# barbararoessle/e2e_multi_view_matching

Hardware: NVIDIA H100
Metric: view-tuples/sec @1024 kpts 5-view (higher is better)
Workload: dtype f32 via split operands on the tensor cores (fp16x3 / tf32x3, fp32-faithful) / f64 pose kernels

## Files before the change

### e2e_multi_view_matching_b200/csrc/attention_h3.cu

```cuda
#include "attention_wg.cuh"

int g_attn_h3_variant = 1;
extern "C" void mvm_debug_set_attention_h3_variant(int v) { g_attn_h3_variant = v ? 1 : 0; }

int launch_attention_h3(const float* qkv, const __half* kh, const __half* kl, const __half* vh, const __half* vl,
                        float* out, int batch, int n_pad, AttnSegs segs, int is_cross, cudaStream_t stream) {
  MVM_REQUIRE(qkv && kh && kl && vh && vl && out);
  MVM_REQUIRE(n_pad % 64 == 0 && attn_segs_valid(segs, n_pad, is_cross));
  MvmProfScope prof__(MVM_TAG_ATTN, stream);
  const long long rows = (long long)batch * segs.n_views * n_pad;
  const CUtensorMap* tK = mvm_get_tmap_2d_f16(kh, rows, 256, 256, attn_wg::BKV);
  const CUtensorMap* tKlo = mvm_get_tmap_2d_f16(kl, rows, 256, 256, attn_wg::BKV);
  const CUtensorMap* tV = mvm_get_tmap_2d_f16(vh, rows, 256, 256, attn_wg::BKV);
  const CUtensorMap* tVlo = mvm_get_tmap_2d_f16(vl, rows, 256, 256, attn_wg::BKV);
  return attn_wg::launch<16>(tK, tV, tKlo, tVlo, qkv, out, batch, n_pad, segs, is_cross, stream);
}
```

### e2e_multi_view_matching_b200/csrc/attention_tc.cu

```cuda
#include "attention_wg.cuh"

long long* g_attn_dbg = nullptr;

extern "C" void mvm_debug_set_attention_timing(long long* buf) { g_attn_dbg = buf; }

int launch_attention_tc(const float* qkv, const float* vt, float* out, int batch, int n_pad, AttnSegs segs,
                        int is_cross, int n_pass, cudaStream_t stream, const float* klo, const float* vtlo) {
  MVM_REQUIRE(n_pad % 64 == 0 && attn_segs_valid(segs, n_pad, is_cross));
  MvmProfScope prof__(MVM_TAG_ATTN, stream);
  const int V = batch * segs.n_views;
  const long long rows = (long long)V * n_pad;
  const CUtensorMap* tK = mvm_get_tmap_2d(qkv, rows, 768, 768, attn_wg::BKV);
  const CUtensorMap* tV = mvm_get_tmap_2d(vt, (long long)V * 256, n_pad, n_pad, attn_wg::HD);
  if (n_pass == 3) {
    MVM_REQUIRE(klo && vtlo);
    const CUtensorMap* tKlo = mvm_get_tmap_2d(klo, rows, 256, 256, attn_wg::BKV);
    const CUtensorMap* tVlo = mvm_get_tmap_2d(vtlo, (long long)V * 256, n_pad, n_pad, attn_wg::HD);
    return attn_wg::launch<3>(tK, tV, tKlo, tVlo, qkv, out, batch, n_pad, segs, is_cross, stream);
  }
  return attn_wg::launch<1>(tK, tV, tK, tV, qkv, out, batch, n_pad, segs, is_cross, stream);
}
```

### e2e_multi_view_matching_b200/csrc/attention_wg.cuh

```cuda
#pragma once
#include <cuda_fp16.h>
#include "common.cuh"
#include "kernels.cuh"
#include "tc_common.cuh"

namespace attn_wg {

constexpr int BQ = 128, BKV = 64, HD = 64;
constexpr int NTHREADS = 288;
constexpr int PRODUCER_WARP = 8;
constexpr int PP_BAR = 1, Q_BAR = 3;

template <int MODE>
struct Cfg {
  static constexpr bool F16 = MODE == 16;
  static constexpr bool PIPE = F16;
  static constexpr int PL = MODE == 1 ? 1 : 2;
  static constexpr int PLANE = F16 ? 8192 : 16384;
  static constexpr int TILE = PL * PLANE;
  static constexpr int ST = MODE == 3 ? 3 : 4;
  static constexpr int OFF_V = ST * TILE;
  static constexpr int OFF_Q = 2 * ST * TILE;
  static constexpr int QPLANE = BQ * 128;
  static constexpr int OFF_BAR = OFF_Q + (F16 ? 2 * QPLANE : 0);
  static constexpr int SMEM_BYTES = OFF_BAR + 256 + 1024;
};

struct Args {
  const float* qkv;
  float* out;
  int n_pad;
  AttnSegs segs;
  int is_cross;
};

__device__ __forceinline__ float ex2_ftz(float x) {
  float y;
  asm("ex2.approx.ftz.f32 %0, %1;" : "=f"(y) : "f"(x));
  return y;
}
__device__ __forceinline__ float tf32_hi(float x) {
  return __uint_as_float((__float_as_uint(x) + 0x1000u) & 0xffffe000u);
}
__device__ __forceinline__ void split_pack(float x0, float x1, uint32_t& hi, uint32_t& lo) {
  const __half2 h = __floats2half2_rn(x0, x1);
  const float2 hf = __half22float2(h);
  const __half2 l = __floats2half2_rn(x0 - hf.x, x1 - hf.y);
  hi = *reinterpret_cast<const uint32_t*>(&h);
  lo = *reinterpret_cast<const uint32_t*>(&l);
}
__device__ __forceinline__ void named_bar_sync(int id, int n) {
  asm volatile("bar.sync %0, %1;" ::"r"(id), "r"(n) : "memory");
}
__device__ __forceinline__ void named_bar_arrive(int id, int n) {
  asm volatile("bar.arrive %0, %1;" ::"r"(id), "r"(n) : "memory");
}
template <int N>
__device__ __forceinline__ void fence_regs(uint32_t (*a)[4]) {
#pragma unroll
  for (int i = 0; i < N; ++i)
#pragma unroll
    for (int e = 0; e < 4; ++e) asm volatile("" : "+r"(a[i][e])::"memory");
}

template <int MODE>
__global__ void __launch_bounds__(NTHREADS, 1)
attention_wg_kernel(const __grid_constant__ CUtensorMap tmK, const __grid_constant__ CUtensorMap tmV,
                    const __grid_constant__ CUtensorMap tmKlo, const __grid_constant__ CUtensorMap tmVlo,
                    const __grid_constant__ Args g) {
  using C_ = Cfg<MODE>;
  constexpr bool F16 = C_::F16, PIPE = C_::PIPE;
  constexpr int ST = C_::ST, PLANE = C_::PLANE, TILE = C_::TILE;
  constexpr int KS = F16 ? 4 : 8;
  extern __shared__ uint8_t smem_raw[];
  uint8_t* smem = reinterpret_cast<uint8_t*>((reinterpret_cast<uintptr_t>(smem_raw) + 1023) & ~uintptr_t(1023));
  uint64_t* bars = reinterpret_cast<uint64_t*>(smem + C_::OFF_BAR);
  uint64_t* k_full = bars;
  uint64_t* k_empty = bars + ST;
  uint64_t* v_full = bars + 2 * ST;
  uint64_t* v_empty = bars + 3 * ST;

  const int warp = threadIdx.x >> 5, lane = threadIdx.x & 31;
  const int q0 = blockIdx.x * BQ;
  const int h = blockIdx.y;
  const int v = blockIdx.z;
  const int T = g.segs.n_views;
  const int t = v % T, b = v / T;
  if (q0 >= g.segs.counts[t]) return;

  if (threadIdx.x == 0) {
    for (int i = 0; i < ST; ++i) {
      tc::mbar_init(k_full + i, 1); tc::mbar_init(k_empty + i, 256);
      tc::mbar_init(v_full + i, 1); tc::mbar_init(v_empty + i, 256);
    }
    tc::fence_barrier_init();
  }
  __syncthreads();

  if (warp == PRODUCER_WARP) {
    if (lane == 0) {
      tc::prefetch_tmap(&tmK); tc::prefetch_tmap(&tmV);
      if (MODE != 1) { tc::prefetch_tmap(&tmKlo); tc::prefetch_tmap(&tmVlo); }
      int j = 0;
      for (int sg = 0; sg < T; ++sg) {
        if (g.is_cross ? (sg == t) : (sg != t)) continue;
        const int cnt = g.segs.counts[sg];
        for (int k0 = 0; k0 < cnt; k0 += BKV, ++j) {
          const int s = j % ST;
          const uint32_t ph = ((j / ST) & 1) ^ 1;
          const int krow = (b * T + sg) * g.n_pad + k0;
          uint8_t* sk = smem + s * TILE;
          uint8_t* sv = smem + C_::OFF_V + s * TILE;
          tc::mbar_wait(k_empty + s, ph);
          tc::mbar_arrive_expect_tx(k_full + s, TILE);
          if (F16) {
            tc::tma_load_2d(sk, &tmK, k_full + s, h * HD, krow);
            tc::tma_load_2d(sk + PLANE, &tmKlo, k_full + s, h * HD, krow);
          } else {
            tc::tma_load_2d(sk, &tmK, k_full + s, 256 + h * HD, krow);
            tc::tma_load_2d(sk + 8192, &tmK, k_full + s, 256 + h * HD + 32, krow);
            if (MODE == 3) {
              tc::tma_load_2d(sk + PLANE, &tmKlo, k_full + s, h * HD, krow);
              tc::tma_load_2d(sk + PLANE + 8192, &tmKlo, k_full + s, h * HD + 32, krow);
            }
          }
          tc::mbar_wait(v_empty + s, ph);
          tc::mbar_arrive_expect_tx(v_full + s, TILE);
          if (F16) {
            tc::tma_load_2d(sv, &tmV, v_full + s, h * HD, krow);
            tc::tma_load_2d(sv + PLANE, &tmVlo, v_full + s, h * HD, krow);
          } else {
            const int vrow = (b * T + sg) * 256 + h * HD;
            tc::tma_load_2d(sv, &tmV, v_full + s, k0, vrow);
            tc::tma_load_2d(sv + 8192, &tmV, v_full + s, k0 + 32, vrow);
            if (MODE == 3) {
              tc::tma_load_2d(sv + PLANE, &tmVlo, v_full + s, k0, vrow);
              tc::tma_load_2d(sv + PLANE + 8192, &tmVlo, v_full + s, k0 + 32, vrow);
            }
          }
        }
      }
    }
    return;
  }

  const int wg = warp >> 2, wq = warp & 3;
  const int gr = lane >> 2, tq = lane & 3;
  const int lrow = wg * 64 + wq * 16 + gr;
  float2 qraw[KS][4];
  {
    const long long total = (long long)gridDim.z * g.n_pad;
    const long long r0 = (long long)v * g.n_pad + q0 + lrow;
    const float* q_r0 = g.qkv + r0 * 768 + h * HD;
    const float* q_r1 = q_r0 + 8 * 768;
    const bool in0 = r0 < total, in1 = r0 + 8 < total;
    const float2 z = make_float2(0.f, 0.f);
#pragma unroll
    for (int kk = 0; kk < KS; ++kk) {
      if (F16) {
        const int c = 16 * kk + 2 * tq;
        qraw[kk][0] = in0 ? __ldg(reinterpret_cast<const float2*>(q_r0 + c)) : z;
        qraw[kk][1] = in1 ? __ldg(reinterpret_cast<const float2*>(q_r1 + c)) : z;
        qraw[kk][2] = in0 ? __ldg(reinterpret_cast<const float2*>(q_r0 + c + 8)) : z;
        qraw[kk][3] = in1 ? __ldg(reinterpret_cast<const float2*>(q_r1 + c + 8)) : z;
      } else {
        const int c = 8 * kk + tq;
        qraw[kk][0] = make_float2(in0 ? __ldg(q_r0 + c) : 0.f, 0.f);
        qraw[kk][1] = make_float2(in1 ? __ldg(q_r1 + c) : 0.f, 0.f);
        qraw[kk][2] = make_float2(in0 ? __ldg(q_r0 + c + 4) : 0.f, 0.f);
        qraw[kk][3] = make_float2(in1 ? __ldg(q_r1 + c + 4) : 0.f, 0.f);
      }
    }
  }
  if constexpr (F16) {
    uint8_t* sq = smem + C_::OFF_Q + lrow * 128 + 4 * tq;
#pragma unroll
    for (int kk = 0; kk < KS; ++kk) {
#pragma unroll
      for (int e = 0; e < 4; ++e) {
        uint32_t hi, lo;
        split_pack(qraw[kk][e].x, qraw[kk][e].y, hi, lo);
        const int off = (e & 1) * 1024 + (((2 * kk + (e >> 1)) ^ gr) << 4);
        *reinterpret_cast<uint32_t*>(sq + off) = hi;
        *reinterpret_cast<uint32_t*>(sq + C_::QPLANE + off) = lo;
      }
    }
    tc::fence_proxy_async();
    named_bar_sync(Q_BAR + wg, 128);
  }

  float o[32];
#pragma unroll
  for (int i = 0; i < 32; ++i) o[i] = 0.f;
  float m_run[2] = {-INFINITY, -INFINITY}, l_run[2] = {0.f, 0.f};
  const float scale_l2e = 0.125f * 1.4426950408889634f;
  const int srcA = (lane & ~3) | (tq >> 1), srcB = srcA + 2;
  float sc[32], fo[2];
  uint32_t qhi[KS][4], qlo[KS][4];
  uint32_t phi[KS][4], plo[KS][4];

  auto prep_s = [&] {
    if constexpr (!F16) {
#pragma unroll
      for (int kk = 0; kk < KS; ++kk) {
#pragma unroll
        for (int e = 0; e < 4; ++e) {
          float x = qraw[kk][e].x;
          asm volatile("" : "+f"(x));
          const float hi = MODE == 3 ? tf32_hi(x) : x;
          qhi[kk][e] = __float_as_uint(hi);
          qlo[kk][e] = __float_as_uint(MODE == 3 ? tf32_hi(x - hi) : 0.f);
        }
      }
    }
#pragma unroll
    for (int i = 0; i < 32; ++i) sc[i] = 0.f;
    tc::fence_acc<64>(sc);
  };
  auto issue_s = [&](int st, uint32_t ph) {
    tc::mbar_wait(k_full + st, ph);
    const uint32_t kb = tc::smem_u32(smem + st * TILE);
    tc::wgmma_fence();
#pragma unroll
    for (int kk = 0; kk < KS; ++kk) {
      if (F16) {
        const uint32_t qb = tc::smem_u32(smem + C_::OFF_Q + wg * 64 * 128) + kk * 32;
        const uint64_t dq = tc::make_sw128_desc(qb), dk = tc::make_sw128_desc(kb + kk * 32);
        tc::wgmma_f16_ss<64>(sc, dq, dk);
        tc::wgmma_f16_ss<64>(sc, dq, tc::make_sw128_desc(kb + PLANE + kk * 32));
        tc::wgmma_f16_ss<64>(sc, tc::make_sw128_desc(qb + C_::QPLANE), dk);
      } else {
        const uint32_t off = (kk >> 2) * 8192 + (kk & 3) * 32;
        const uint64_t dk = tc::make_sw128_desc(kb + off);
        tc::wgmma_tf32_rs<64>(sc, qhi[kk], dk);
        if (MODE == 3) {
          tc::wgmma_tf32_rs<64>(sc, qhi[kk], tc::make_sw128_desc(kb + PLANE + off));
          tc::wgmma_tf32_rs<64>(sc, qlo[kk], dk);
        }
      }
    }
    tc::wgmma_commit();
  };
  auto retire_s = [&](int st) {
    tc::fence_acc<64>(sc);
    if constexpr (!F16) { fence_regs<KS>(qhi); fence_regs<KS>(qlo); }
    tc::mbar_arrive(k_empty + st);
  };
  auto issue_pv = [&](int st, uint32_t ph) {
    tc::mbar_wait(v_full + st, ph);
    const uint32_t vb = tc::smem_u32(smem + C_::OFF_V + st * TILE);
    tc::wgmma_fence();
#pragma unroll
    for (int kk = 0; kk < KS; ++kk) {
      if (F16) {
        const uint64_t dv = tc::make_sw128_desc(vb + kk * 2048);
        tc::wgmma_f16_rs<64, 1>(o, phi[kk], dv);
        tc::wgmma_f16_rs<64, 1>(o, phi[kk], tc::make_sw128_desc(vb + PLANE + kk * 2048));
        tc::wgmma_f16_rs<64, 1>(o, plo[kk], dv);
      } else {
        const uint32_t off = (kk >> 2) * 8192 + (kk & 3) * 32;
        const uint64_t dv = tc::make_sw128_desc(vb + off);
        tc::wgmma_tf32_rs<64>(o, phi[kk], dv);
        if (MODE == 3) {
          tc::wgmma_tf32_rs<64>(o, phi[kk], tc::make_sw128_desc(vb + PLANE + off));
          tc::wgmma_tf32_rs<64>(o, plo[kk], dv);
        }
      }
    }
    tc::wgmma_commit();
  };
  auto retire_pv = [&](int st) {
    tc::fence_acc<64>(o);
    fence_regs<KS>(phi);
    fence_regs<KS>(plo);
    tc::mbar_arrive(v_empty + st);
  };
  auto softmax = [&](int nvalid) {
    if (nvalid < BKV) {
#pragma unroll
      for (int i = 0; i < 8; ++i) {
        const int key = 8 * i + 2 * tq;
        if (key >= nvalid) { sc[4 * i] = -INFINITY; sc[4 * i + 2] = -INFINITY; }
        if (key + 1 >= nvalid) { sc[4 * i + 1] = -INFINITY; sc[4 * i + 3] = -INFINITY; }
      }
    }
#pragma unroll
    for (int hh = 0; hh < 2; ++hh) {
      float mx = sc[2 * hh];
#pragma unroll
      for (int i = 0; i < 8; ++i) mx = fmaxf(mx, fmaxf(sc[4 * i + 2 * hh], sc[4 * i + 2 * hh + 1]));
      mx = fmaxf(mx, __shfl_xor_sync(0xffffffffu, mx, 1));
      mx = fmaxf(mx, __shfl_xor_sync(0xffffffffu, mx, 2));
      mx *= scale_l2e;
      fo[hh] = 1.f;
      if (mx > m_run[hh] + 8.f) {
        fo[hh] = ex2_ftz(m_run[hh] - mx);
        m_run[hh] = mx;
        l_run[hh] *= fo[hh];
      }
      const float nm = 7.f - m_run[hh];
      float rs = 0.f;
#pragma unroll
      for (int i = 0; i < 8; ++i) {
        const float p0 = ex2_ftz(fmaf(sc[4 * i + 2 * hh], scale_l2e, nm));
        const float p1 = ex2_ftz(fmaf(sc[4 * i + 2 * hh + 1], scale_l2e, nm));
        sc[4 * i + 2 * hh] = p0;
        sc[4 * i + 2 * hh + 1] = p1;
        rs += p0 + p1;
      }
      l_run[hh] += rs;
    }
  };
  auto rescale_o = [&] {
#pragma unroll
    for (int hh = 0; hh < 2; ++hh) {
      if (fo[hh] != 1.f) {
#pragma unroll
        for (int i = 0; i < 8; ++i) {
          o[4 * i + 2 * hh] *= fo[hh];
          o[4 * i + 2 * hh + 1] *= fo[hh];
        }
      }
    }
  };
  auto split_p = [&] {
#pragma unroll
    for (int kk = 0; kk < KS; ++kk) {
      if (F16) {
#pragma unroll
        for (int e = 0; e < 4; ++e) split_pack(sc[8 * kk + 2 * e], sc[8 * kk + 2 * e + 1], phi[kk][e], plo[kk][e]);
      } else {
        float a[4];
        const bool odd = tq & 1;
        const float x0 = __shfl_sync(0xffffffffu, sc[4 * kk], srcA), x1 = __shfl_sync(0xffffffffu, sc[4 * kk + 1], srcA);
        const float y0 = __shfl_sync(0xffffffffu, sc[4 * kk + 2], srcA), y1 = __shfl_sync(0xffffffffu, sc[4 * kk + 3], srcA);
        const float z0 = __shfl_sync(0xffffffffu, sc[4 * kk], srcB), z1 = __shfl_sync(0xffffffffu, sc[4 * kk + 1], srcB);
        const float w0 = __shfl_sync(0xffffffffu, sc[4 * kk + 2], srcB), w1 = __shfl_sync(0xffffffffu, sc[4 * kk + 3], srcB);
        a[0] = odd ? x1 : x0; a[1] = odd ? y1 : y0; a[2] = odd ? z1 : z0; a[3] = odd ? w1 : w0;
#pragma unroll
        for (int e = 0; e < 4; ++e) {
          const float hi = MODE == 3 ? tf32_hi(a[e]) : a[e];
          phi[kk][e] = __float_as_uint(hi);
          plo[kk][e] = __float_as_uint(a[e] - hi);
        }
      }
    }
  };

  auto finish_pv = [&](int jn) {
    tc::wgmma_wait<0>();
    tc::fence_acc<64>(o);
    fence_regs<KS>(phi);
    fence_regs<KS>(plo);
    if (jn >= 2) tc::mbar_arrive(v_empty + (jn - 2) % ST);
    if (jn >= 1) {
      rescale_o();
      split_p();
    }
  };
  if (PIPE && wg == 1) named_bar_arrive(PP_BAR + 0, 256);
  int j = 0;
  for (int sg = 0; sg < T; ++sg) {
    if (g.is_cross ? (sg == t) : (sg != t)) continue;
    const int cnt = g.segs.counts[sg];
    for (int k0 = 0; k0 < cnt; k0 += BKV, ++j) {
      const int nvalid = cnt - k0;
      const int s = j % ST;
      const uint32_t ph = (j / ST) & 1;
      if constexpr (PIPE) {
        finish_pv(j);
        prep_s();
        named_bar_sync(PP_BAR + wg, 256);
        if (j == 0) {
          issue_s(s, ph);
          named_bar_arrive(PP_BAR + (wg ^ 1), 256);
          tc::wgmma_wait<0>();
        } else {
          issue_s(s, ph);
          issue_pv((j - 1) % ST, ((j - 1) / ST) & 1);
          named_bar_arrive(PP_BAR + (wg ^ 1), 256);
          tc::wgmma_wait<1>();
        }
        retire_s(s);
        softmax(nvalid);
      } else {
        prep_s();
        issue_s(s, ph);
        tc::wgmma_wait<0>();
        retire_s(s);
        softmax(nvalid);
        rescale_o();
        split_p();
        issue_pv(s, ph);
        tc::wgmma_wait<0>();
        retire_pv(s);
      }
    }
  }
  if constexpr (PIPE) {
    finish_pv(j);
    named_bar_sync(PP_BAR + wg, 256);
    if (j > 0) issue_pv((j - 1) % ST, ((j - 1) / ST) & 1);
    if (wg == 0) named_bar_arrive(PP_BAR + 1, 256);
    tc::wgmma_wait<0>();
    if (j > 0) retire_pv((j - 1) % ST);
  }

#pragma unroll
  for (int hh = 0; hh < 2; ++hh) {
    float l = l_run[hh];
    l += __shfl_xor_sync(0xffffffffu, l, 1);
    l += __shfl_xor_sync(0xffffffffu, l, 2);
    const float inv = 1.f / l;
    const int r = lrow + 8 * hh;
    if (q0 + r < g.n_pad) {
      float* op = g.out + ((long long)v * g.n_pad + q0 + r) * 256 + h * HD + 2 * tq;
#pragma unroll
      for (int i = 0; i < 8; ++i)
        *reinterpret_cast<float2*>(op + 8 * i) = make_float2(o[4 * i + 2 * hh] * inv, o[4 * i + 2 * hh + 1] * inv);
    }
  }
}

template <int MODE>
int launch(const CUtensorMap* tK, const CUtensorMap* tV, const CUtensorMap* tKlo, const CUtensorMap* tVlo, const float* qkv,
           float* out, int batch, int n_pad, const AttnSegs& segs, int is_cross, cudaStream_t stream) {
  using C_ = Cfg<MODE>;
  if (!tK || !tV || !tKlo || !tVlo) return MVM_ERR_LAUNCH;
  mvm_once_per_device(MODE == 16 ? MVM_ONCE_ATTN_H3 : MVM_ONCE_ATTN_TC + 16 * (MODE == 3), [&] {
    cudaFuncSetAttribute(attention_wg_kernel<MODE>, cudaFuncAttributeMaxDynamicSharedMemorySize, C_::SMEM_BYTES);
  });
  Args g;
  g.qkv = qkv; g.out = out; g.n_pad = n_pad; g.segs = segs; g.is_cross = is_cross;
  dim3 grid(mvm_div_up(n_pad, BQ), 4, batch * segs.n_views);
  attention_wg_kernel<MODE><<<grid, NTHREADS, C_::SMEM_BYTES, stream>>>(*tK, *tV, *tKlo, *tVlo, g);
  MVM_CHECK_LAUNCH();
  return MVM_OK;
}

}
```

### e2e_multi_view_matching_b200/csrc/tc_common.cuh

```cuda
#pragma once
#include <cuda.h>
#include <cuda_runtime.h>
#include <stdint.h>

namespace tc {

__device__ __forceinline__ uint32_t smem_u32(const void* p) {
  return static_cast<uint32_t>(__cvta_generic_to_shared(p));
}

__device__ __forceinline__ void mbar_init(uint64_t* bar, uint32_t count) {
  asm volatile("mbarrier.init.shared::cta.b64 [%0], %1;" ::"r"(smem_u32(bar)), "r"(count));
}
__device__ __forceinline__ void fence_barrier_init() {
  asm volatile("fence.mbarrier_init.release.cluster;" ::: "memory");
}
__device__ __forceinline__ void fence_proxy_async() {
  asm volatile("fence.proxy.async.shared::cta;" ::: "memory");
}
__device__ __forceinline__ void mbar_arrive_expect_tx(uint64_t* bar, uint32_t bytes) {
  asm volatile("mbarrier.arrive.expect_tx.shared::cta.b64 _, [%0], %1;" ::"r"(smem_u32(bar)), "r"(bytes)
               : "memory");
}
__device__ __forceinline__ void mbar_arrive(uint64_t* bar) {
  asm volatile("mbarrier.arrive.shared::cta.b64 _, [%0];" ::"r"(smem_u32(bar)) : "memory");
}
__device__ __forceinline__ void mbar_wait(uint64_t* bar, uint32_t parity) {
  const uint32_t addr = smem_u32(bar);
  asm volatile(
      "{\n\t"
      ".reg .pred P1;\n\t"
      "WAIT_LOOP:\n\t"
      "mbarrier.try_wait.parity.shared::cta.b64 P1, [%0], %1;\n\t"
      "@P1 bra DONE;\n\t"
      "bra WAIT_LOOP;\n\t"
      "DONE:\n\t"
      "}" ::"r"(addr),
      "r"(parity)
      : "memory");
}

__device__ __forceinline__ void prefetch_tmap(const CUtensorMap* m) {
  asm volatile("prefetch.tensormap [%0];" ::"l"(reinterpret_cast<uint64_t>(m)) : "memory");
}
__device__ __forceinline__ void tma_load_2d(void* dst, const CUtensorMap* m, uint64_t* bar, int c0, int c1) {
  asm volatile(
      "cp.async.bulk.tensor.2d.shared::cluster.global.tile.mbarrier::complete_tx::bytes [%0], [%1, {%3, %4}], [%2];"
      ::"r"(smem_u32(dst)), "l"(reinterpret_cast<uint64_t>(m)), "r"(smem_u32(bar)), "r"(c0), "r"(c1)
      : "memory");
}
__device__ __forceinline__ void tma_load_3d(void* dst, const CUtensorMap* m, uint64_t* bar, int c0, int c1,
                                            int c2) {
  asm volatile(
      "cp.async.bulk.tensor.3d.shared::cluster.global.tile.mbarrier::complete_tx::bytes [%0], [%1, {%3, %4, %5}], [%2];"
      ::"r"(smem_u32(dst)), "l"(reinterpret_cast<uint64_t>(m)), "r"(smem_u32(bar)), "r"(c0), "r"(c1), "r"(c2)
      : "memory");
}

__device__ __forceinline__ void tma_store_2d(const CUtensorMap* m, const void* src, int c0, int c1) {
  asm volatile("cp.async.bulk.tensor.2d.global.shared::cta.tile.bulk_group [%0, {%2, %3}], [%1];"
               ::"l"(reinterpret_cast<uint64_t>(m)), "r"(smem_u32(src)), "r"(c0), "r"(c1)
               : "memory");
}
__device__ __forceinline__ void tma_store_commit() { asm volatile("cp.async.bulk.commit_group;" ::: "memory"); }
template <int N>
__device__ __forceinline__ void tma_store_wait_read() {
  asm volatile("cp.async.bulk.wait_group.read %0;" ::"n"(N) : "memory");
}
__device__ __forceinline__ void tma_store_wait_all() { asm volatile("cp.async.bulk.wait_group 0;" ::: "memory"); }

__device__ __forceinline__ uint64_t make_sw128_desc(uint32_t smem_addr) {
  uint64_t d = 0;
  d |= static_cast<uint64_t>((smem_addr & 0x3FFFF) >> 4);
  d |= static_cast<uint64_t>(1) << 16;
  d |= static_cast<uint64_t>(1024 >> 4) << 32;
  d |= static_cast<uint64_t>(1) << 62;
  return d;
}
__device__ __forceinline__ void wgmma_fence() { asm volatile("wgmma.fence.sync.aligned;" ::: "memory"); }
__device__ __forceinline__ void wgmma_commit() { asm volatile("wgmma.commit_group.sync.aligned;" ::: "memory"); }
template <int N>
__device__ __forceinline__ void wgmma_wait() { asm volatile("wgmma.wait_group.sync.aligned %0;" ::"n"(N) : "memory"); }
template <int N>
__device__ __forceinline__ void fence_acc(float* d) {
#pragma unroll
  for (int i = 0; i < N / 2; ++i) asm volatile("" : "+f"(d[i])::"memory");
}

template <int N> __device__ __forceinline__ void wgmma_tf32_rs(float* d, const uint32_t* a, uint64_t bdesc);
template <int N, int TB> __device__ __forceinline__ void wgmma_f16_rs(float* d, const uint32_t* a, uint64_t bdesc);
template <> __device__ __forceinline__ void wgmma_tf32_rs<64>(float* d, const uint32_t* a, uint64_t bdesc) {
  asm volatile(
      "{\n\t.reg .pred p;\n\tsetp.eq.u32 p, 1, 1;\n\t"
      "wgmma.mma_async.sync.aligned.m64n64k8.f32.tf32.tf32 "
      "{%0, %1, %2, %3, %4, %5, %6, %7, %8, %9, %10, %11, %12, %13, %14, %15, %16, %17, %18, %19, %20, %21, %22, %23, %24, %25, %26, %27, %28, %29, %30, %31}, {%32, %33, %34, %35}, %36, p, 1, 1;\n\t}"
      : "+f"(d[0]), "+f"(d[1]), "+f"(d[2]), "+f"(d[3]), "+f"(d[4]), "+f"(d[5]), "+f"(d[6]), "+f"(d[7]), "+f"(d[8]), "+f"(d[9]), "+f"(d[10]), "+f"(d[11]), "+f"(d[12]), "+f"(d[13]), "+f"(d[14]), "+f"(d[15]), "+f"(d[16]), "+f"(d[17]), "+f"(d[18]), "+f"(d[19]), "+f"(d[20]), "+f"(d[21]), "+f"(d[22]), "+f"(d[23]), "+f"(d[24]), "+f"(d[25]), "+f"(d[26]), "+f"(d[27]), "+f"(d[28]), "+f"(d[29]), "+f"(d[30]), "+f"(d[31])
      : "r"(a[0]), "r"(a[1]), "r"(a[2]), "r"(a[3]), "l"(bdesc));
}
template <> __device__ __forceinline__ void wgmma_f16_rs<64, 0>(float* d, const uint32_t* a, uint64_t bdesc) {
  asm volatile(
      "{\n\t.reg .pred p;\n\tsetp.eq.u32 p, 1, 1;\n\t"
      "wgmma.mma_async.sync.aligned.m64n64k16.f32.f16.f16 "
      "{%0, %1, %2, %3, %4, %5, %6, %7, %8, %9, %10, %11, %12, %13, %14, %15, %16, %17, %18, %19, %20, %21, %22, %23, %24, %25, %26, %27, %28, %29, %30, %31}, {%32, %33, %34, %35}, %36, p, 1, 1, 0;\n\t}"
      : "+f"(d[0]), "+f"(d[1]), "+f"(d[2]), "+f"(d[3]), "+f"(d[4]), "+f"(d[5]), "+f"(d[6]), "+f"(d[7]), "+f"(d[8]), "+f"(d[9]), "+f"(d[10]), "+f"(d[11]), "+f"(d[12]), "+f"(d[13]), "+f"(d[14]), "+f"(d[15]), "+f"(d[16]), "+f"(d[17]), "+f"(d[18]), "+f"(d[19]), "+f"(d[20]), "+f"(d[21]), "+f"(d[22]), "+f"(d[23]), "+f"(d[24]), "+f"(d[25]), "+f"(d[26]), "+f"(d[27]), "+f"(d[28]), "+f"(d[29]), "+f"(d[30]), "+f"(d[31])
      : "r"(a[0]), "r"(a[1]), "r"(a[2]), "r"(a[3]), "l"(bdesc));
}
template <> __device__ __forceinline__ void wgmma_f16_rs<64, 1>(float* d, const uint32_t* a, uint64_t bdesc) {
  asm volatile(
      "{\n\t.reg .pred p;\n\tsetp.eq.u32 p, 1, 1;\n\t"
      "wgmma.mma_async.sync.aligned.m64n64k16.f32.f16.f16 "
      "{%0, %1, %2, %3, %4, %5, %6, %7, %8, %9, %10, %11, %12, %13, %14, %15, %16, %17, %18, %19, %20, %21, %22, %23, %24, %25, %26, %27, %28, %29, %30, %31}, {%32, %33, %34, %35}, %36, p, 1, 1, 1;\n\t}"
      : "+f"(d[0]), "+f"(d[1]), "+f"(d[2]), "+f"(d[3]), "+f"(d[4]), "+f"(d[5]), "+f"(d[6]), "+f"(d[7]), "+f"(d[8]), "+f"(d[9]), "+f"(d[10]), "+f"(d[11]), "+f"(d[12]), "+f"(d[13]), "+f"(d[14]), "+f"(d[15]), "+f"(d[16]), "+f"(d[17]), "+f"(d[18]), "+f"(d[19]), "+f"(d[20]), "+f"(d[21]), "+f"(d[22]), "+f"(d[23]), "+f"(d[24]), "+f"(d[25]), "+f"(d[26]), "+f"(d[27]), "+f"(d[28]), "+f"(d[29]), "+f"(d[30]), "+f"(d[31])
      : "r"(a[0]), "r"(a[1]), "r"(a[2]), "r"(a[3]), "l"(bdesc));
}
template <> __device__ __forceinline__ void wgmma_tf32_rs<128>(float* d, const uint32_t* a, uint64_t bdesc) {
  asm volatile(
      "{\n\t.reg .pred p;\n\tsetp.eq.u32 p, 1, 1;\n\t"
      "wgmma.mma_async.sync.aligned.m64n128k8.f32.tf32.tf32 "
      "{%0, %1, %2, %3, %4, %5, %6, %7, %8, %9, %10, %11, %12, %13, %14, %15, %16, %17, %18, %19, %20, %21, %22, %23, %24, %25, %26, %27, %28, %29, %30, %31, %32, %33, %34, %35, %36, %37, %38, %39, %40, %41, %42, %43, %44, %45, %46, %47, %48, %49, %50, %51, %52, %53, %54, %55, %56, %57, %58, %59, %60, %61, %62, %63}, {%64, %65, %66, %67}, %68, p, 1, 1;\n\t}"
      : "+f"(d[0]), "+f"(d[1]), "+f"(d[2]), "+f"(d[3]), "+f"(d[4]), "+f"(d[5]), "+f"(d[6]), "+f"(d[7]), "+f"(d[8]), "+f"(d[9]), "+f"(d[10]), "+f"(d[11]), "+f"(d[12]), "+f"(d[13]), "+f"(d[14]), "+f"(d[15]), "+f"(d[16]), "+f"(d[17]), "+f"(d[18]), "+f"(d[19]), "+f"(d[20]), "+f"(d[21]), "+f"(d[22]), "+f"(d[23]), "+f"(d[24]), "+f"(d[25]), "+f"(d[26]), "+f"(d[27]), "+f"(d[28]), "+f"(d[29]), "+f"(d[30]), "+f"(d[31]), "+f"(d[32]), "+f"(d[33]), "+f"(d[34]), "+f"(d[35]), "+f"(d[36]), "+f"(d[37]), "+f"(d[38]), "+f"(d[39]), "+f"(d[40]), "+f"(d[41]), "+f"(d[42]), "+f"(d[43]), "+f"(d[44]), "+f"(d[45]), "+f"(d[46]), "+f"(d[47]), "+f"(d[48]), "+f"(d[49]), "+f"(d[50]), "+f"(d[51]), "+f"(d[52]), "+f"(d[53]), "+f"(d[54]), "+f"(d[55]), "+f"(d[56]), "+f"(d[57]), "+f"(d[58]), "+f"(d[59]), "+f"(d[60]), "+f"(d[61]), "+f"(d[62]), "+f"(d[63])
      : "r"(a[0]), "r"(a[1]), "r"(a[2]), "r"(a[3]), "l"(bdesc));
}
template <> __device__ __forceinline__ void wgmma_f16_rs<128, 0>(float* d, const uint32_t* a, uint64_t bdesc) {
  asm volatile(
      "{\n\t.reg .pred p;\n\tsetp.eq.u32 p, 1, 1;\n\t"
      "wgmma.mma_async.sync.aligned.m64n128k16.f32.f16.f16 "
      "{%0, %1, %2, %3, %4, %5, %6, %7, %8, %9, %10, %11, %12, %13, %14, %15, %16, %17, %18, %19, %20, %21, %22, %23, %24, %25, %26, %27, %28, %29, %30, %31, %32, %33, %34, %35, %36, %37, %38, %39, %40, %41, %42, %43, %44, %45, %46, %47, %48, %49, %50, %51, %52, %53, %54, %55, %56, %57, %58, %59, %60, %61, %62, %63}, {%64, %65, %66, %67}, %68, p, 1, 1, 0;\n\t}"
      : "+f"(d[0]), "+f"(d[1]), "+f"(d[2]), "+f"(d[3]), "+f"(d[4]), "+f"(d[5]), "+f"(d[6]), "+f"(d[7]), "+f"(d[8]), "+f"(d[9]), "+f"(d[10]), "+f"(d[11]), "+f"(d[12]), "+f"(d[13]), "+f"(d[14]), "+f"(d[15]), "+f"(d[16]), "+f"(d[17]), "+f"(d[18]), "+f"(d[19]), "+f"(d[20]), "+f"(d[21]), "+f"(d[22]), "+f"(d[23]), "+f"(d[24]), "+f"(d[25]), "+f"(d[26]), "+f"(d[27]), "+f"(d[28]), "+f"(d[29]), "+f"(d[30]), "+f"(d[31]), "+f"(d[32]), "+f"(d[33]), "+f"(d[34]), "+f"(d[35]), "+f"(d[36]), "+f"(d[37]), "+f"(d[38]), "+f"(d[39]), "+f"(d[40]), "+f"(d[41]), "+f"(d[42]), "+f"(d[43]), "+f"(d[44]), "+f"(d[45]), "+f"(d[46]), "+f"(d[47]), "+f"(d[48]), "+f"(d[49]), "+f"(d[50]), "+f"(d[51]), "+f"(d[52]), "+f"(d[53]), "+f"(d[54]), "+f"(d[55]), "+f"(d[56]), "+f"(d[57]), "+f"(d[58]), "+f"(d[59]), "+f"(d[60]), "+f"(d[61]), "+f"(d[62]), "+f"(d[63])
      : "r"(a[0]), "r"(a[1]), "r"(a[2]), "r"(a[3]), "l"(bdesc));
}
template <> __device__ __forceinline__ void wgmma_f16_rs<128, 1>(float* d, const uint32_t* a, uint64_t bdesc) {
  asm volatile(
      "{\n\t.reg .pred p;\n\tsetp.eq.u32 p, 1, 1;\n\t"
      "wgmma.mma_async.sync.aligned.m64n128k16.f32.f16.f16 "
      "{%0, %1, %2, %3, %4, %5, %6, %7, %8, %9, %10, %11, %12, %13, %14, %15, %16, %17, %18, %19, %20, %21, %22, %23, %24, %25, %26, %27, %28, %29, %30, %31, %32, %33, %34, %35, %36, %37, %38, %39, %40, %41, %42, %43, %44, %45, %46, %47, %48, %49, %50, %51, %52, %53, %54, %55, %56, %57, %58, %59, %60, %61, %62, %63}, {%64, %65, %66, %67}, %68, p, 1, 1, 1;\n\t}"
      : "+f"(d[0]), "+f"(d[1]), "+f"(d[2]), "+f"(d[3]), "+f"(d[4]), "+f"(d[5]), "+f"(d[6]), "+f"(d[7]), "+f"(d[8]), "+f"(d[9]), "+f"(d[10]), "+f"(d[11]), "+f"(d[12]), "+f"(d[13]), "+f"(d[14]), "+f"(d[15]), "+f"(d[16]), "+f"(d[17]), "+f"(d[18]), "+f"(d[19]), "+f"(d[20]), "+f"(d[21]), "+f"(d[22]), "+f"(d[23]), "+f"(d[24]), "+f"(d[25]), "+f"(d[26]), "+f"(d[27]), "+f"(d[28]), "+f"(d[29]), "+f"(d[30]), "+f"(d[31]), "+f"(d[32]), "+f"(d[33]), "+f"(d[34]), "+f"(d[35]), "+f"(d[36]), "+f"(d[37]), "+f"(d[38]), "+f"(d[39]), "+f"(d[40]), "+f"(d[41]), "+f"(d[42]), "+f"(d[43]), "+f"(d[44]), "+f"(d[45]), "+f"(d[46]), "+f"(d[47]), "+f"(d[48]), "+f"(d[49]), "+f"(d[50]), "+f"(d[51]), "+f"(d[52]), "+f"(d[53]), "+f"(d[54]), "+f"(d[55]), "+f"(d[56]), "+f"(d[57]), "+f"(d[58]), "+f"(d[59]), "+f"(d[60]), "+f"(d[61]), "+f"(d[62]), "+f"(d[63])
      : "r"(a[0]), "r"(a[1]), "r"(a[2]), "r"(a[3]), "l"(bdesc));
}
template <int N> __device__ __forceinline__ void wgmma_f16_ss(float* d, uint64_t adesc, uint64_t bdesc);
template <> __device__ __forceinline__ void wgmma_f16_ss<64>(float* d, uint64_t adesc, uint64_t bdesc) {
  asm volatile(
      "{\n\t.reg .pred p;\n\tsetp.eq.u32 p, 1, 1;\n\t"
      "wgmma.mma_async.sync.aligned.m64n64k16.f32.f16.f16 "
      "{%0, %1, %2, %3, %4, %5, %6, %7, %8, %9, %10, %11, %12, %13, %14, %15, %16, %17, %18, %19, %20, %21, %22, %23, %24, %25, %26, %27, %28, %29, %30, %31}, %32, %33, p, 1, 1, 0, 0;\n\t}"
      : "+f"(d[0]), "+f"(d[1]), "+f"(d[2]), "+f"(d[3]), "+f"(d[4]), "+f"(d[5]), "+f"(d[6]), "+f"(d[7]), "+f"(d[8]), "+f"(d[9]), "+f"(d[10]), "+f"(d[11]), "+f"(d[12]), "+f"(d[13]), "+f"(d[14]), "+f"(d[15]), "+f"(d[16]), "+f"(d[17]), "+f"(d[18]), "+f"(d[19]), "+f"(d[20]), "+f"(d[21]), "+f"(d[22]), "+f"(d[23]), "+f"(d[24]), "+f"(d[25]), "+f"(d[26]), "+f"(d[27]), "+f"(d[28]), "+f"(d[29]), "+f"(d[30]), "+f"(d[31])
      : "l"(adesc), "l"(bdesc));
}


__device__ __forceinline__ float tf32_rn(float x) {
  uint32_t r;
  asm("cvt.rna.tf32.f32 %0, %1;" : "=r"(r) : "f"(x));
  return __uint_as_float(r);
}

}

const CUtensorMap* mvm_get_tmap_2d(const float* base, long long rows, long long cols, long long ld, int box_rows);
const CUtensorMap* mvm_get_tmap_2d_f16(const void* base, long long rows, long long cols, long long ld, int box_rows);

const CUtensorMap* mvm_get_tmap_3d(const float* base, long long slabs, long long rows, long long cols,
                                   long long ld_row, long long ld_slab, int box_rows);
```

Measured before the change: 192.4.

## Widen fp16 attention KV tile to 128, keep Q in registers, rebalance registers

The fp16x3 attention path now uses 128-key tiles instead of 64 and feeds Q hi/lo to wgmma straight from registers (RS form) rather than staging it in shared memory. The producer group becomes a full warpgroup that gives up registers via setmaxnreg so the consumers can hold 232 registers. This is meant to halve the per-tile barrier and softmax overhead, free the Q shared-memory planes, and remove the Q staging barrier. The costs are larger score accumulators, which raise register pressure and spill risk, a shallower pipeline (3 stages instead of 4), and more idle producer threads.

```diff
diff --git a/e2e_multi_view_matching_b200/csrc/attention_h3.cu b/e2e_multi_view_matching_b200/csrc/attention_h3.cu
--- a/e2e_multi_view_matching_b200/csrc/attention_h3.cu
+++ b/e2e_multi_view_matching_b200/csrc/attention_h3.cu
@@ -9,9 +9,9 @@
   MVM_REQUIRE(n_pad % 64 == 0 && attn_segs_valid(segs, n_pad, is_cross));
   MvmProfScope prof__(MVM_TAG_ATTN, stream);
   const long long rows = (long long)batch * segs.n_views * n_pad;
-  const CUtensorMap* tK = mvm_get_tmap_2d_f16(kh, rows, 256, 256, attn_wg::BKV);
-  const CUtensorMap* tKlo = mvm_get_tmap_2d_f16(kl, rows, 256, 256, attn_wg::BKV);
-  const CUtensorMap* tV = mvm_get_tmap_2d_f16(vh, rows, 256, 256, attn_wg::BKV);
-  const CUtensorMap* tVlo = mvm_get_tmap_2d_f16(vl, rows, 256, 256, attn_wg::BKV);
+  const CUtensorMap* tK = mvm_get_tmap_2d_f16(kh, rows, 256, 256, attn_wg::Cfg<16>::BKV);
+  const CUtensorMap* tKlo = mvm_get_tmap_2d_f16(kl, rows, 256, 256, attn_wg::Cfg<16>::BKV);
+  const CUtensorMap* tV = mvm_get_tmap_2d_f16(vh, rows, 256, 256, attn_wg::Cfg<16>::BKV);
+  const CUtensorMap* tVlo = mvm_get_tmap_2d_f16(vl, rows, 256, 256, attn_wg::Cfg<16>::BKV);
   return attn_wg::launch<16>(tK, tV, tKlo, tVlo, qkv, out, batch, n_pad, segs, is_cross, stream);
 }
diff --git a/e2e_multi_view_matching_b200/csrc/attention_tc.cu b/e2e_multi_view_matching_b200/csrc/attention_tc.cu
--- a/e2e_multi_view_matching_b200/csrc/attention_tc.cu
+++ b/e2e_multi_view_matching_b200/csrc/attention_tc.cu
@@ -10,11 +10,11 @@
   MvmProfScope prof__(MVM_TAG_ATTN, stream);
   const int V = batch * segs.n_views;
   const long long rows = (long long)V * n_pad;
-  const CUtensorMap* tK = mvm_get_tmap_2d(qkv, rows, 768, 768, attn_wg::BKV);
+  const CUtensorMap* tK = mvm_get_tmap_2d(qkv, rows, 768, 768, attn_wg::Cfg<1>::BKV);
   const CUtensorMap* tV = mvm_get_tmap_2d(vt, (long long)V * 256, n_pad, n_pad, attn_wg::HD);
   if (n_pass == 3) {
     MVM_REQUIRE(klo && vtlo);
-    const CUtensorMap* tKlo = mvm_get_tmap_2d(klo, rows, 256, 256, attn_wg::BKV);
+    const CUtensorMap* tKlo = mvm_get_tmap_2d(klo, rows, 256, 256, attn_wg::Cfg<1>::BKV);
     const CUtensorMap* tVlo = mvm_get_tmap_2d(vtlo, (long long)V * 256, n_pad, n_pad, attn_wg::HD);
     return attn_wg::launch<3>(tK, tV, tKlo, tVlo, qkv, out, batch, n_pad, segs, is_cross, stream);
   }
diff --git a/e2e_multi_view_matching_b200/csrc/attention_wg.cuh b/e2e_multi_view_matching_b200/csrc/attention_wg.cuh
--- a/e2e_multi_view_matching_b200/csrc/attention_wg.cuh
+++ b/e2e_multi_view_matching_b200/csrc/attention_wg.cuh
@@ -6,23 +6,23 @@
 
 namespace attn_wg {
 
-constexpr int BQ = 128, BKV = 64, HD = 64;
-constexpr int NTHREADS = 288;
+constexpr int BQ = 128, HD = 64;
 constexpr int PRODUCER_WARP = 8;
-constexpr int PP_BAR = 1, Q_BAR = 3;
+constexpr int NTHREADS = 384;
+constexpr int PRODUCER_REGS = 40, CONSUMER_REGS = 232;
+constexpr int PP_BAR = 1;
 
 template <int MODE>
 struct Cfg {
   static constexpr bool F16 = MODE == 16;
   static constexpr bool PIPE = F16;
+  static constexpr int BKV = F16 ? 128 : 64;
   static constexpr int PL = MODE == 1 ? 1 : 2;
-  static constexpr int PLANE = F16 ? 8192 : 16384;
+  static constexpr int PLANE = 16384;
   static constexpr int TILE = PL * PLANE;
-  static constexpr int ST = MODE == 3 ? 3 : 4;
+  static constexpr int ST = MODE == 1 ? 4 : 3;
   static constexpr int OFF_V = ST * TILE;
-  static constexpr int OFF_Q = 2 * ST * TILE;
-  static constexpr int QPLANE = BQ * 128;
-  static constexpr int OFF_BAR = OFF_Q + (F16 ? 2 * QPLANE : 0);
+  static constexpr int OFF_BAR = 2 * ST * TILE;
   static constexpr int SMEM_BYTES = OFF_BAR + 256 + 1024;
 };
 
@@ -70,8 +70,10 @@
                     const __grid_constant__ Args g) {
   using C_ = Cfg<MODE>;
   constexpr bool F16 = C_::F16, PIPE = C_::PIPE;
-  constexpr int ST = C_::ST, PLANE = C_::PLANE, TILE = C_::TILE;
+  constexpr int ST = C_::ST, PLANE = C_::PLANE, TILE = C_::TILE, BKV = C_::BKV;
   constexpr int KS = F16 ? 4 : 8;
+  constexpr int KP = BKV / (F16 ? 16 : 8);
+  constexpr int NSC = BKV / 2;
   extern __shared__ uint8_t smem_raw[];
   uint8_t* smem = reinterpret_cast<uint8_t*>((reinterpret_cast<uintptr_t>(smem_raw) + 1023) & ~uintptr_t(1023));
   uint64_t* bars = reinterpret_cast<uint64_t*>(smem + C_::OFF_BAR);
@@ -97,8 +99,9 @@
   }
   __syncthreads();
 
-  if (warp == PRODUCER_WARP) {
-    if (lane == 0) {
+  if (warp >= PRODUCER_WARP) {
+    asm volatile("setmaxnreg.dec.sync.aligned.u32 %0;" ::"n"(PRODUCER_REGS));
+    if (warp == PRODUCER_WARP && lane == 0) {
       tc::prefetch_tmap(&tmK); tc::prefetch_tmap(&tmV);
       if (MODE != 1) { tc::prefetch_tmap(&tmKlo); tc::prefetch_tmap(&tmVlo); }
       int j = 0;
@@ -144,6 +147,7 @@
     return;
   }
 
+  asm volatile("setmaxnreg.inc.sync.aligned.u32 %0;" ::"n"(CONSUMER_REGS));
   const int wg = warp >> 2, wq = warp & 3;
   const int gr = lane >> 2, tq = lane & 3;
   const int lrow = wg * 64 + wq * 16 + gr;
@@ -172,21 +176,12 @@
       }
     }
   }
+  uint32_t qhi[KS][4], qlo[KS][4];
   if constexpr (F16) {
-    uint8_t* sq = smem + C_::OFF_Q + lrow * 128 + 4 * tq;
-#pragma unroll
-    for (int kk = 0; kk < KS; ++kk) {
-#pragma unroll
-      for (int e = 0; e < 4; ++e) {
-        uint32_t hi, lo;
-        split_pack(qraw[kk][e].x, qraw[kk][e].y, hi, lo);
-        const int off = (e & 1) * 1024 + (((2 * kk + (e >> 1)) ^ gr) << 4);
-        *reinterpret_cast<uint32_t*>(sq + off) = hi;
-        *reinterpret_cast<uint32_t*>(sq + C_::QPLANE + off) = lo;
-      }
-    }
-    tc::fence_proxy_async();
-    named_bar_sync(Q_BAR + wg, 128);
+#pragma unroll
+    for (int kk = 0; kk < KS; ++kk)
+#pragma unroll
+      for (int e = 0; e < 4; ++e) split_pack(qraw[kk][e].x, qraw[kk][e].y, qhi[kk][e], qlo[kk][e]);
   }
 
   float o[32];
@@ -195,9 +190,8 @@
   float m_run[2] = {-INFINITY, -INFINITY}, l_run[2] = {0.f, 0.f};
   const float scale_l2e = 0.125f * 1.4426950408889634f;
   const int srcA = (lane & ~3) | (tq >> 1), srcB = srcA + 2;
-  float sc[32], fo[2];
-  uint32_t qhi[KS][4], qlo[KS][4];
-  uint32_t phi[KS][4], plo[KS][4];
+  float sc[NSC], fo[2];
+  uint32_t phi[KP][4], plo[KP][4];
 
   auto prep_s = [&] {
     if constexpr (!F16) {
@@ -214,8 +208,8 @@
       }
     }
 #pragma unroll
-    for (int i = 0; i < 32; ++i) sc[i] = 0.f;
-    tc::fence_acc<64>(sc);
+    for (int i = 0; i < NSC; ++i) sc[i] = 0.f;
+    tc::fence_acc<BKV>(sc);
   };
   auto issue_s = [&](int st, uint32_t ph) {
     tc::mbar_wait(k_full + st, ph);
@@ -224,11 +218,10 @@
 #pragma unroll
     for (int kk = 0; kk < KS; ++kk) {
       if (F16) {
-        const uint32_t qb = tc::smem_u32(smem + C_::OFF_Q + wg * 64 * 128) + kk * 32;
-        const uint64_t dq = tc::make_sw128_desc(qb), dk = tc::make_sw128_desc(kb + kk * 32);
-        tc::wgmma_f16_ss<64>(sc, dq, dk);
-        tc::wgmma_f16_ss<64>(sc, dq, tc::make_sw128_desc(kb + PLANE + kk * 32));
-        tc::wgmma_f16_ss<64>(sc, tc::make_sw128_desc(qb + C_::QPLANE), dk);
+        const uint64_t dk = tc::make_sw128_desc(kb + kk * 32);
+        tc::wgmma_f16_rs<BKV, 0>(sc, qhi[kk], dk);
+        tc::wgmma_f16_rs<BKV, 0>(sc, qhi[kk], tc::make_sw128_desc(kb + PLANE + kk * 32));
+        tc::wgmma_f16_rs<BKV, 0>(sc, qlo[kk], dk);
       } else {
         const uint32_t off = (kk >> 2) * 8192 + (kk & 3) * 32;
         const uint64_t dk = tc::make_sw128_desc(kb + off);
@@ -242,8 +235,9 @@
     tc::wgmma_commit();
   };
   auto retire_s = [&](int st) {
-    tc::fence_acc<64>(sc);
-    if constexpr (!F16) { fence_regs<KS>(qhi); fence_regs<KS>(qlo); }
+    tc::fence_acc<BKV>(sc);
+    fence_regs<KS>(qhi);
+    fence_regs<KS>(qlo);
     tc::mbar_arrive(k_empty + st);
   };
   auto issue_pv = [&](int st, uint32_t ph) {
@@ -251,7 +245,7 @@
     const uint32_t vb = tc::smem_u32(smem + C_::OFF_V + st * TILE);
     tc::wgmma_fence();
 #pragma unroll
-    for (int kk = 0; kk < KS; ++kk) {
+    for (int kk = 0; kk < KP; ++kk) {
       if (F16) {
         const uint64_t dv = tc::make_sw128_desc(vb + kk * 2048);
         tc::wgmma_f16_rs<64, 1>(o, phi[kk], dv);
@@ -271,14 +265,14 @@
   };
   auto retire_pv = [&](int st) {
     tc::fence_acc<64>(o);
-    fence_regs<KS>(phi);
-    fence_regs<KS>(plo);
+    fence_regs<KP>(phi);
+    fence_regs<KP>(plo);
     tc::mbar_arrive(v_empty + st);
   };
   auto softmax = [&](int nvalid) {
     if (nvalid < BKV) {
 #pragma unroll
-      for (int i = 0; i < 8; ++i) {
+      for (int i = 0; i < BKV / 8; ++i) {
         const int key = 8 * i + 2 * tq;
         if (key >= nvalid) { sc[4 * i] = -INFINITY; sc[4 * i + 2] = -INFINITY; }
         if (key + 1 >= nvalid) { sc[4 * i + 1] = -INFINITY; sc[4 * i + 3] = -INFINITY; }
@@ -288,7 +282,7 @@
     for (int hh = 0; hh < 2; ++hh) {
       float mx = sc[2 * hh];
 #pragma unroll
-      for (int i = 0; i < 8; ++i) mx = fmaxf(mx, fmaxf(sc[4 * i + 2 * hh], sc[4 * i + 2 * hh + 1]));
+      for (int i = 0; i < BKV / 8; ++i) mx = fmaxf(mx, fmaxf(sc[4 * i + 2 * hh], sc[4 * i + 2 * hh + 1]));
       mx = fmaxf(mx, __shfl_xor_sync(0xffffffffu, mx, 1));
       mx = fmaxf(mx, __shfl_xor_sync(0xffffffffu, mx, 2));
       mx *= scale_l2e;
@@ -301,7 +295,7 @@
       const float nm = 7.f - m_run[hh];
       float rs = 0.f;
 #pragma unroll
-      for (int i = 0; i < 8; ++i) {
+      for (int i = 0; i < BKV / 8; ++i) {
         const float p0 = ex2_ftz(fmaf(sc[4 * i + 2 * hh], scale_l2e, nm));
         const float p1 = ex2_ftz(fmaf(sc[4 * i + 2 * hh + 1], scale_l2e, nm));
         sc[4 * i + 2 * hh] = p0;
@@ -325,7 +319,7 @@
   };
   auto split_p = [&] {
 #pragma unroll
-    for (int kk = 0; kk < KS; ++kk) {
+    for (int kk = 0; kk < KP; ++kk) {
       if (F16) {
 #pragma unroll
         for (int e = 0; e < 4; ++e) split_pack(sc[8 * kk + 2 * e], sc[8 * kk + 2 * e + 1], phi[kk][e], plo[kk][e]);
@@ -350,8 +344,8 @@
   auto finish_pv = [&](int jn) {
     tc::wgmma_wait<0>();
     tc::fence_acc<64>(o);
-    fence_regs<KS>(phi);
-    fence_regs<KS>(plo);
+    fence_regs<KP>(phi);
+    fence_regs<KP>(plo);
     if (jn >= 2) tc::mbar_arrive(v_empty + (jn - 2) % ST);
     if (jn >= 1) {
       rescale_o();
diff --git a/e2e_multi_view_matching_b200/csrc/tc_common.cuh b/e2e_multi_view_matching_b200/csrc/tc_common.cuh
--- a/e2e_multi_view_matching_b200/csrc/tc_common.cuh
+++ b/e2e_multi_view_matching_b200/csrc/tc_common.cuh
@@ -137,16 +137,6 @@
       : "+f"(d[0]), "+f"(d[1]), "+f"(d[2]), "+f"(d[3]), "+f"(d[4]), "+f"(d[5]), "+f"(d[6]), "+f"(d[7]), "+f"(d[8]), "+f"(d[9]), "+f"(d[10]), "+f"(d[11]), "+f"(d[12]), "+f"(d[13]), "+f"(d[14]), "+f"(d[15]), "+f"(d[16]), "+f"(d[17]), "+f"(d[18]), "+f"(d[19]), "+f"(d[20]), "+f"(d[21]), "+f"(d[22]), "+f"(d[23]), "+f"(d[24]), "+f"(d[25]), "+f"(d[26]), "+f"(d[27]), "+f"(d[28]), "+f"(d[29]), "+f"(d[30]), "+f"(d[31]), "+f"(d[32]), "+f"(d[33]), "+f"(d[34]), "+f"(d[35]), "+f"(d[36]), "+f"(d[37]), "+f"(d[38]), "+f"(d[39]), "+f"(d[40]), "+f"(d[41]), "+f"(d[42]), "+f"(d[43]), "+f"(d[44]), "+f"(d[45]), "+f"(d[46]), "+f"(d[47]), "+f"(d[48]), "+f"(d[49]), "+f"(d[50]), "+f"(d[51]), "+f"(d[52]), "+f"(d[53]), "+f"(d[54]), "+f"(d[55]), "+f"(d[56]), "+f"(d[57]), "+f"(d[58]), "+f"(d[59]), "+f"(d[60]), "+f"(d[61]), "+f"(d[62]), "+f"(d[63])
       : "r"(a[0]), "r"(a[1]), "r"(a[2]), "r"(a[3]), "l"(bdesc));
 }
-template <int N> __device__ __forceinline__ void wgmma_f16_ss(float* d, uint64_t adesc, uint64_t bdesc);
-template <> __device__ __forceinline__ void wgmma_f16_ss<64>(float* d, uint64_t adesc, uint64_t bdesc) {
-  asm volatile(
-      "{\n\t.reg .pred p;\n\tsetp.eq.u32 p, 1, 1;\n\t"
-      "wgmma.mma_async.sync.aligned.m64n64k16.f32.f16.f16 "
-      "{%0, %1, %2, %3, %4, %5, %6, %7, %8, %9, %10, %11, %12, %13, %14, %15, %16, %17, %18, %19, %20, %21, %22, %23, %24, %25, %26, %27, %28, %29, %30, %31}, %32, %33, p, 1, 1, 0, 0;\n\t}"
-      : "+f"(d[0]), "+f"(d[1]), "+f"(d[2]), "+f"(d[3]), "+f"(d[4]), "+f"(d[5]), "+f"(d[6]), "+f"(d[7]), "+f"(d[8]), "+f"(d[9]), "+f"(d[10]), "+f"(d[11]), "+f"(d[12]), "+f"(d[13]), "+f"(d[14]), "+f"(d[15]), "+f"(d[16]), "+f"(d[17]), "+f"(d[18]), "+f"(d[19]), "+f"(d[20]), "+f"(d[21]), "+f"(d[22]), "+f"(d[23]), "+f"(d[24]), "+f"(d[25]), "+f"(d[26]), "+f"(d[27]), "+f"(d[28]), "+f"(d[29]), "+f"(d[30]), "+f"(d[31])
-      : "l"(adesc), "l"(bdesc));
-}
-
 
 __device__ __forceinline__ float tf32_rn(float x) {
   uint32_t r;
```

Result: faster. 201.0, median of 6 (+4.5%).
